# dusk-network/jubjub-schnorr

Measured on AMD Instinct MI355X. Metric: Schnorr verifications/sec, higher is better.
Workload: dtype u32 limbs (29-bit), u64 accumulators

## Files before the change

### jubjub_schnorr_amd/csrc/ed29.h

```cpp
#pragma once
#include "fq29.h"

namespace jjs {

using fe_t = fe<1, 5>;

struct ext_pt {
    fe_n x, y, z, t;
};
struct niels_pt {
    fe_t ypx, ymx, z, t2d;
};

JJS_HD fe_n fe_n_one() { return fq_as<1, 2>(fq_one()); }
JJS_HD fe_n fe_n_zero() { return fq_as<1, 2>(fq_zero()); }

JJS_HD ext_pt ext_identity() {
    ext_pt p;
    p.x = fe_n_zero(); p.y = fe_n_one(); p.z = fe_n_one(); p.t = fe_n_zero();
    return p;
}
JJS_HD ext_pt ext_from_affine(const fe_n& u, const fe_n& v) {
    ext_pt p;
    p.x = u; p.y = v; p.z = fe_n_one(); p.t = fq_mul(u, v);
    return p;
}
JJS_HD niels_pt niels_identity() {
    niels_pt n;
    n.ypx = fq_as<1, 5>(fq_one()); n.ymx = n.ypx; n.z = n.ypx; n.t2d = fq_as<1, 5>(fq_zero());
    return n;
}
JJS_HD niels_pt to_niels(const ext_pt& p) {
    niels_pt n;
    n.ypx = fq_as<1, 5>(fq_norm(fq_add(p.y, p.x)));
    n.ymx = fq_norm(fq_sub(p.y, p.x));
    n.z = fq_as<1, 5>(p.z);
    n.t2d = fq_as<1, 5>(fq_mul(p.t, fe_from_const<1, 1>(JJS_D2)));
    return n;
}
JJS_HD niels_pt niels_select(bool c, const niels_pt& a, const niels_pt& b) {
    niels_pt r;
    r.ypx = fq_select(c, a.ypx, b.ypx); r.ymx = fq_select(c, a.ymx, b.ymx);
    r.z = fq_select(c, a.z, b.z); r.t2d = fq_select(c, a.t2d, b.t2d);
    return r;
}

JJS_HD ext_pt ext_double(const ext_pt& p, bool need_t) {
    auto e = fq_dbl(fq_mul_hot(p.x, p.y));
    fe_n xx = fq_sqr_hot(p.x);
    fe_n yy = fq_sqr_hot(p.y);
    auto c2 = fq_dbl(fq_sqr_hot(p.z));
    auto g = fq_norm(fq_add(yy, xx));
    auto h = fq_sub(yy, xx);
    auto f = fq_norm(fq_sub(fq_add(c2, xx), yy));
    ext_pt r;
    r.x = fq_mul_hot(e, f);
    r.z = fq_mul_hot(f, h);
    r.y = fq_mul_hot(h, g);
    if (need_t) r.t = fq_mul_hot(g, e); else r.t = fe_n_zero();
    return r;
}

JJS_HD ext_pt ext_add_niels(const ext_pt& p, const niels_pt& n, bool neg, bool need_t) {
    fe_t n_ymx = fq_select(neg, n.ypx, n.ymx);
    fe_t n_ypx = fq_select(neg, n.ymx, n.ypx);
    auto n_t2d = fq_select(neg, fq_neg(n.t2d), fq_as<2, 6>(n.t2d));
    fe_n a = fq_mul_hot(fq_sub(p.y, p.x), n_ymx);
    fe_n b = fq_mul_hot(fq_add(p.y, p.x), n_ypx);
    fe_n c = fq_mul_hot(p.t, n_t2d);
    auto d = fq_dbl(fq_mul_hot(p.z, n.z));
    auto e = fq_sub(b, a);
    auto f = fq_norm(fq_sub(d, c));
    auto g = fq_add(d, c);
    auto h = fq_norm(fq_add(b, a));
    ext_pt r;
    r.x = fq_mul_hot(e, f);
    r.z = fq_mul_hot(f, g);
    r.y = fq_mul_hot(g, h);
    if (need_t) r.t = fq_mul_hot(h, e); else r.t = fe_n_zero();
    return r;
}
JJS_HD ext_pt ext_add_affine_niels(const ext_pt& p, const fe_t& n_ypx, const fe_t& n_ymx, const fe_t& n_t2d,
                                   bool need_t) {
    fe_n a = fq_mul_hot(fq_sub(p.y, p.x), n_ymx);
    fe_n b = fq_mul_hot(fq_add(p.y, p.x), n_ypx);
    fe_n c = fq_mul_hot(p.t, n_t2d);
    auto d = fq_dbl(p.z);
    auto e = fq_sub(b, a);
    auto f = fq_norm(fq_sub(d, c));
    auto g = fq_add(d, c);
    auto h = fq_norm(fq_add(b, a));
    ext_pt r;
    r.x = fq_mul_hot(e, f);
    r.z = fq_mul_hot(f, g);
    r.y = fq_mul_hot(g, h);
    if (need_t) r.t = fq_mul_hot(h, e); else r.t = fe_n_zero();
    return r;
}

JJS_HD bool ext_is_identity(const ext_pt& p) { return fq_is_zero(p.x) && fq_eq(p.y, p.z); }

JJS_HD bool affine_on_curve(const fe_n& u, const fe_n& v) {
    fe_n u2 = fq_sqr(u), v2 = fq_sqr(v);
    auto lhs = fq_sub(v2, u2);
    auto rhs = fq_norm(fq_add(fq_mul(fq_mul(u2, v2), fe_from_const<1, 1>(JJS_D)), fq_one()));
    return fq_eq(lhs, rhs);
}
JJS_HD bool affine_is_identity(const fe_n& u, const fe_n& v) { return fq_is_zero(u) && fq_eq(v, fq_one()); }

JJS_HD bool ext_eq_affine(const ext_pt& p, const fe_n& u, const fe_n& v) {
    return fq_eq(p.x, fq_mul(u, p.z)) && fq_eq(p.y, fq_mul(v, p.z));
}

}
```

### jubjub_schnorr_amd/csrc/jjs_constants.inc

```
#define JJS_MAX_HASH_INPUTS 16
#define JJS_Q29_0 0x00000001u
#define JJS_Q29_1 0x1ffffff8u
#define JJS_Q29_2 0x1f96ffbfu
#define JJS_Q29_3 0x1b4805ffu
#define JJS_Q29_4 0x1d80553bu
#define JJS_Q29_5 0x0c0404d0u
#define JJS_Q29_6 0x1520cce7u
#define JJS_Q29_7 0x0a6533afu
#define JJS_Q29_8 0x0073eda7u
JJS_CONST uint32_t JJS_Q_WORDS[8] = {0x00000001u, 0xffffffffu, 0xfffe5bfeu, 0x53bda402u, 0x09a1d805u, 0x3339d808u, 0x299d7d48u, 0x73eda753u};
JJS_CONST uint32_t JJS_QM2_WORDS[8] = {0xffffffffu, 0xfffffffeu, 0xfffe5bfeu, 0x53bda402u, 0x09a1d805u, 0x3339d808u, 0x299d7d48u, 0x73eda753u};
JJS_CONST uint32_t JJS_FR_WORDS[8] = {0xd6f72cb7u, 0xd0970e5eu, 0xccc81082u, 0xa6682093u, 0x01343b00u, 0x06673b01u, 0x6533afa9u, 0x0e7db4eau};
JJS_CONST uint32_t JJS_FR_R2_WORDS[8] = {0x95e57731u, 0x67719aa4u, 0x9ce3fc26u, 0x51b0cef0u, 0xc026e9a5u, 0x69dab7fau, 0x8d127688u, 0x04f6547bu};
#define JJS_FR_INV32 0xef788ef9u
JJS_CONST uint32_t JJS_R2[9] = {0x0a71b3c0u, 0x1d32207eu, 0x1663d999u, 0x1c5abc93u, 0x03b58c44u, 0x0be37438u, 0x0829f771u, 0x1660139eu, 0x0027fd91u};
JJS_CONST uint32_t JJS_ONE[9] = {0x1fffffbau, 0x0000022fu, 0x1cb61180u, 0x0a4e5c00u, 0x0ee8b1a2u, 0x16e6aedfu, 0x1907f8bbu, 0x0853ddf7u, 0x004d043fu};
JJS_CONST uint32_t JJS_D[9] = {0x0e9ed5e8u, 0x12245679u, 0x002d9f52u, 0x03bb3367u, 0x0d9bfb3du, 0x18ebb3ccu, 0x1c29ceccu, 0x0a7b6020u, 0x0020d725u};
JJS_CONST uint32_t JJS_D2[9] = {0x1d3dabd0u, 0x0448acf2u, 0x005b3ea5u, 0x077666ceu, 0x1b37f67au, 0x11d76798u, 0x18539d99u, 0x14f6c041u, 0x0041ae4au};
JJS_CONST uint32_t JJS_G[2][9] = {{0x0f8e352bu, 0x0d898cfcu, 0x1acf8b86u, 0x11cbaed5u, 0x11f53f06u, 0x1e102b0eu, 0x1a54d9c6u, 0x143eceffu, 0x006815d6u}, {0x1ffffb09u, 0x000027b7u, 0x09503dc0u, 0x0d6a3610u, 0x07d8d3d7u, 0x180c16bcu, 0x1a26af41u, 0x038c62dfu, 0x006f1642u}};
JJS_CONST uint32_t JJS_GN[2][9] = {{0x187d023du, 0x137e7289u, 0x0690434eu, 0x1f76361du, 0x00cee7a6u, 0x0f6ffe89u, 0x0eae76dcu, 0x0b002f63u, 0x001b3c2eu}, {0x0d19dfe5u, 0x1ba2bfe4u, 0x0aa87077u, 0x0a3c12aeu, 0x0f209d38u, 0x03331d80u, 0x05e964c7u, 0x046d436du, 0x00027722u}};
JJS_CONST uint32_t JJS_DOUBLE_TAG_WORDS[8] = {0x4844424cu, 0x4a4a5343u, 0x00000000u, 0x00000000u, 0x00000000u, 0x00000000u, 0x00000000u, 0x00000000u};
JJS_CONST uint32_t JJS_SPONGE_TAG[JJS_MAX_HASH_INPUTS + 1][9] = {
  {0x00000000u, 0x00000000u, 0x00000000u, 0x00000000u, 0x00000000u, 0x00000000u, 0x00000000u, 0x00000000u, 0x00000000u},
  {0x0505ee08u, 0x1a263c20u, 0x0be84b8bu, 0x14a02c49u, 0x01c71b32u, 0x0119871du, 0x0e158ab3u, 0x1ae4f29eu, 0x002534dfu},
  {0x1b0be909u, 0x1f0bd4a7u, 0x15c76ef6u, 0x19aa6651u, 0x03d277dau, 0x02c51eb8u, 0x131e6edfu, 0x1c823839u, 0x0028ae1cu},
  {0x0fc46418u, 0x0273db7eu, 0x16529079u, 0x104dd318u, 0x168e8637u, 0x026f5725u, 0x1c808eacu, 0x029e0e17u, 0x003fedbdu},
  {0x0357c163u, 0x10043808u, 0x19bdf7a6u, 0x0d30d38fu, 0x12e5297bu, 0x1c58dc5fu, 0x0ba83205u, 0x06d45679u, 0x00090830u},
  {0x0262554eu, 0x06977c58u, 0x1cc4c932u, 0x13bcc122u, 0x0d7d7321u, 0x16c6f8cdu, 0x0c42072du, 0x0a7ba9d5u, 0x00467f10u},
  {0x16ed364au, 0x0b0ae88eu, 0x1bd377f9u, 0x1bebcca6u, 0x0fbf0111u, 0x0eacca90u, 0x174be582u, 0x0d8cb0dfu, 0x006048a8u},
  {0x1648d83cu, 0x1c96a336u, 0x13f93121u, 0x0404c2c5u, 0x12088053u, 0x05063ca4u, 0x1387a958u, 0x0e2ca8b5u, 0x000dc63bu},
  {0x1f8df888u, 0x05a7ef5au, 0x1e8dea4fu, 0x04cf9c40u, 0x03a338cdu, 0x11ce25feu, 0x08f757fcu, 0x197c5746u, 0x00448b3du},
  {0x18861d85u, 0x0bfc90f3u, 0x01a0c7f1u, 0x0b8f8540u, 0x061d8364u, 0x17492b24u, 0x1f89fbceu, 0x03e0f6e4u, 0x002d13cau},
  {0x0f24fc1du, 0x17584430u, 0x197f7236u, 0x1bad9229u, 0x17ce7252u, 0x12745987u, 0x119f85a5u, 0x0365f792u, 0x00419641u},
  {0x0ad4ee1du, 0x1c33dd77u, 0x03cea63au, 0x0090b229u, 0x1eff0500u, 0x1ae3d4a9u, 0x0e58224eu, 0x1ba57ecau, 0x00131c30u},
  {0x0047e885u, 0x12b591deu, 0x09f50887u, 0x0c3877f6u, 0x01adcabbu, 0x00dcbf79u, 0x0ac6f554u, 0x0bcc64deu, 0x0062115cu},
  {0x18868630u, 0x0c3e88d9u, 0x0d12f54du, 0x062083b4u, 0x00efbe4eu, 0x1c915ba8u, 0x11f90d73u, 0x1200490cu, 0x00205cd9u},
  {0x109c52e0u, 0x100352e0u, 0x0d1863ecu, 0x0f9203ccu, 0x08db7deau, 0x1ea7d49cu, 0x0641cbbeu, 0x1693107au, 0x00056607u},
  {0x07380761u, 0x0379c563u, 0x10c89db4u, 0x0924fcebu, 0x0cf29ce1u, 0x1bfecb19u, 0x1a3ca913u, 0x12d81574u, 0x0008852cu},
  {0x0137f8a1u, 0x135b43b9u, 0x1a25c48fu, 0x04e620e0u, 0x0f670a49u, 0x190a832du, 0x1c3afc44u, 0x0c7a93dbu, 0x0026b4abu},
};
JJS_CONST uint32_t JJS_PAIR_L1[2][9] = {{0x1632f828u, 0x1cd998edu, 0x06ef42eau, 0x18522084u, 0x12362748u, 0x02a698c9u, 0x1b29c579u, 0x021b0691u, 0x003c41f3u}, {0x1b06fde4u, 0x137cdc5cu, 0x1714b9b2u, 0x065d7f7du, 0x140f3e68u, 0x08fb5d4bu, 0x18ad857au, 0x02b255c2u, 0x005ac97bu}};
JJS_CONST uint32_t JJS_PAIR_NEG_L2[9] = {0x0ec609f6u, 0x0fa98aa5u, 0x012a02e2u, 0x17e06bfeu, 0x14bb44c6u, 0x0c66138cu, 0x166a4edbu, 0x0ffd0b0au, 0x0050cfe0u};
JJS_CONST uint32_t JJS_PAIR_B[9] = {0x002c2b67u, 0x1e9ea4c8u, 0x07b6263fu, 0x1afbd911u, 0x133cdbc5u, 0x16559828u, 0x1a61d3c3u, 0x10975a2au, 0x00520471u};
JJS_CONST uint32_t JJS_PAIR_EXP_WORDS[8] = {0xe0000000u, 0xdfffffffu, 0x5fffcb7fu, 0xaa77b480u, 0x01343b00u, 0x06673b01u, 0x6533afa9u, 0x0e7db4eau};
#define JJS_PAIR_SW_STEPS 57
#define JJS_PAIR_SW_TRAILING 29
JJS_CONST uint32_t JJS_PAIR_SW[JJS_PAIR_SW_STEPS][2] = {{3, 7}, {5, 7}, {2, 3}, {3, 3}, {3, 3}, {2, 1}, {5, 7}, {4, 5}, {4, 3}, {5, 5}, {4, 3}, {5, 7}, {4, 5}, {3, 7}, {3, 5}, {2, 1}, {3, 1}, {7, 3}, {4, 3}, {5, 7}, {5, 7}, {3, 3}, {8, 1}, {8, 1}, {4, 3}, {2, 1}, {7, 7}, {3, 3}, {11, 5}, {4, 5}, {5, 7}, {4, 7}, {3, 5}, {3, 5}, {3, 1}, {11, 5}, {3, 7}, {3, 7}, {3, 7}, {3, 7}, {2, 3}, {5, 5}, {3, 5}, {3, 7}, {3, 7}, {2, 3}, {4, 7}, {3, 7}, {3, 7}, {3, 7}, {3, 7}, {3, 7}, {3, 7}, {3, 7}, {3, 7}, {3, 7}, {2, 3}};
#define JJS_INV_SW_STEPS 68
#define JJS_INV_SW_TRAILING 0
JJS_CONST uint32_t JJS_INV_SW[JJS_INV_SW_STEPS][2] = {{3, 7}, {5, 7}, {2, 3}, {3, 3}, {3, 3}, {2, 1}, {5, 7}, {4, 5}, {4, 3}, {5, 5}, {4, 3}, {5, 7}, {4, 5}, {3, 7}, {3, 5}, {2, 1}, {3, 1}, {7, 3}, {4, 3}, {5, 7}, {5, 7}, {3, 3}, {8, 1}, {8, 1}, {4, 3}, {2, 1}, {7, 7}, {3, 3}, {11, 5}, {4, 5}, {5, 7}, {4, 7}, {3, 5}, {3, 5}, {3, 1}, {11, 5}, {3, 7}, {3, 7}, {3, 7}, {3, 7}, {2, 3}, {5, 5}, {3, 5}, {3, 7}, {3, 7}, {2, 3}, {4, 7}, {3, 7}, {3, 7}, {3, 7}, {3, 7}, {3, 7}, {3, 7}, {3, 7}, {3, 7}, {3, 7}, {3, 5}, {3, 7}, {3, 7}, {3, 7}, {3, 7}, {3, 7}, {3, 7}, {3, 7}, {3, 7}, {3, 7}, {3, 7}, {1, 1}};
#define JJS_SQRT_SW_STEPS 57
#define JJS_SQRT_SW_TRAILING 0
JJS_CONST uint32_t JJS_SQRT_SW[JJS_SQRT_SW_STEPS][2] = {{3, 7}, {5, 7}, {2, 3}, {3, 3}, {3, 3}, {2, 1}, {5, 7}, {4, 5}, {4, 3}, {5, 5}, {4, 3}, {5, 7}, {4, 5}, {3, 7}, {3, 5}, {2, 1}, {3, 1}, {7, 3}, {4, 3}, {5, 7}, {5, 7}, {3, 3}, {8, 1}, {8, 1}, {4, 3}, {2, 1}, {7, 7}, {3, 3}, {11, 5}, {4, 5}, {5, 7}, {4, 7}, {3, 5}, {3, 5}, {3, 1}, {11, 5}, {3, 7}, {3, 7}, {3, 7}, {3, 7}, {2, 3}, {5, 5}, {3, 5}, {3, 7}, {3, 7}, {2, 3}, {4, 7}, {3, 7}, {3, 7}, {3, 7}, {3, 7}, {3, 7}, {3, 7}, {3, 7}, {3, 7}, {3, 7}, {1, 1}};
JJS_CONST uint32_t JJS_DLOG_BASES[7][9] = {{0x1e643334u, 0x16481b3cu, 0x1b429d12u, 0x177f9dadu, 0x144a8d18u, 0x0d45bdd8u, 0x04734720u, 0x08d7bfb9u, 0x0036d431u}, {0x015b5931u, 0x170bf111u, 0x0fdc692cu, 0x1da57375u, 0x1cd8fb0cu, 0x082b2e9eu, 0x11dae58du, 0x1c3e92cdu, 0x007386deu}, {0x046746cau, 0x011b8fe2u, 0x1ba33a6du, 0x176e1524u, 0x09d99e75u, 0x154d7d8eu, 0x00d23d31u, 0x1df2d37eu, 0x000963afu}, {0x1e643334u, 0x16481b3cu, 0x1b429d12u, 0x177f9dadu, 0x144a8d18u, 0x0d45bdd8u, 0x04734720u, 0x08d7bfb9u, 0x0036d431u}, {0x065b9ba7u, 0x16d68576u, 0x182b2c2au, 0x14d5af02u, 0x07140888u, 0x1362f1d7u, 0x08c77bb2u, 0x1cb1a9c5u, 0x00094bf1u}, {0x1abc62ceu, 0x0fbddb01u, 0x140b0090u, 0x03bc5521u, 0x11f8af58u, 0x1881ae47u, 0x11d5d43eu, 0x0a2d9980u, 0x005fe400u}, {0x04fbdc84u, 0x10c8e2ffu, 0x041d8af4u, 0x1a3da377u, 0x19ceef70u, 0x002b6e41u, 0x0034a007u, 0x1c185b28u, 0x0007ee60u}};
#define JJS_DLOG_HASH_MULT 1u
#define JJS_DLOG_HASH_SHIFT 0
JJS_CONST uint32_t JJS_ROOT_OF_UNITY[9] = {0x01c8cd27u, 0x158d8d27u, 0x19006c0du, 0x09177006u, 0x1b40635eu, 0x01d0b1cau, 0x0d517805u, 0x04859aa2u, 0x002c4064u};
JJS_CONST uint32_t JJS_RC[340][9] = {
  {0x00acd34au, 0x1735f45au, 0x138d6d99u, 0x0ed55d98u, 0x1ca62dc6u, 0x10ba9671u, 0x10435733u, 0x033b644du, 0x004aa8c7u},
  {0x14ffba26u, 0x1ba29e52u, 0x177f0b64u, 0x00b3510cu, 0x127726cfu, 0x1857d2a8u, 0x1e3d168au, 0x15e4d101u, 0x000f1ecau},
  {0x10544837u, 0x105827efu, 0x084c6e15u, 0x0e8aac41u, 0x0ae02b0fu, 0x18ebde5au, 0x0fafaf7cu, 0x083d3281u, 0x0034fd73u},
  {0x0344bf7fu, 0x0a46646au, 0x1730014du, 0x12e0ba85u, 0x02e3906cu, 0x05e7a406u, 0x17f2dc8bu, 0x1945722eu, 0x003a6ecfu},
  {0x1fd22f28u, 0x045b2ea8u, 0x17a649b2u, 0x0f9d7504u, 0x11961944u, 0x1660a34bu, 0x0a6a6237u, 0x193bc629u, 0x0021ffc7u},
  {0x1d29e5b8u, 0x06cae729u, 0x151ba656u, 0x1ac9f0b1u, 0x1b3a5e51u, 0x0d4ca236u, 0x1207ea27u, 0x1d21fa02u, 0x0022dd1fu},
  {0x12400ff9u, 0x0035d81du, 0x03b62299u, 0x025d538au, 0x08e06dddu, 0x1bbf452cu, 0x094dfd08u, 0x00285210u, 0x00308fabu},
  {0x1d184e77u, 0x1592ad1fu, 0x16661d64u, 0x1fe21660u, 0x1bfeebb3u, 0x0b7e4ad3u, 0x17ca297au, 0x15006fa8u, 0x001db197u},
  {0x1ddad3c4u, 0x13a1d246u, 0x071c897bu, 0x164f9a39u, 0x0689f7a5u, 0x080f8889u, 0x135aee92u, 0x03a580b3u, 0x006f4972u},
  {0x0d6eb0dbu, 0x058fde5bu, 0x1499b97cu, 0x0f49db3bu, 0x0ed02c77u, 0x0cd55fdeu, 0x029ef2fbu, 0x1f5282afu, 0x002a2cdcu},
  {0x1ab8ab5fu, 0x027938ecu, 0x0c556f7eu, 0x09fbfaf8u, 0x0ae0ef37u, 0x19cb8097u, 0x0358d657u, 0x12a3f282u, 0x002ebee0u},
  {0x12dd5a05u, 0x1eba6f91u, 0x00b2d3d3u, 0x0aa6ae2cu, 0x13721dbbu, 0x1619de12u, 0x0b03bb30u, 0x1947db06u, 0x000b396bu},
  {0x1f8c17c0u, 0x01352a93u, 0x09e2ed99u, 0x07dac2cdu, 0x0d3aedbeu, 0x053f5f63u, 0x1b33c7e7u, 0x10c2ba42u, 0x0057396bu},
  {0x0e64cfffu, 0x126637e6u, 0x1a0794f9u, 0x1d461805u, 0x01391d16u, 0x1546bc79u, 0x05f70070u, 0x07ffb18du, 0x001842b2u},
  {0x0e764d8au, 0x16095bb4u, 0x0eff26e0u, 0x0b91cc80u, 0x10ecd53du, 0x13e34450u, 0x0ded21a8u, 0x0a797e6eu, 0x00097bc9u},
  {0x1ea10b88u, 0x1f8971a2u, 0x12d7c69du, 0x1ebf9d1bu, 0x0901446fu, 0x001128c0u, 0x12fb8a56u, 0x062dd94au, 0x00133c86u},
  {0x0475856du, 0x0abc329fu, 0x15340d60u, 0x1aad5748u, 0x18d82c8eu, 0x112bd03fu, 0x0968aeabu, 0x1486dedeu, 0x00015fefu},
  {0x1d7537ecu, 0x074ba0f7u, 0x1a721561u, 0x0744501eu, 0x0b007d84u, 0x1f48b991u, 0x05982416u, 0x0db60c99u, 0x00640d9du},
  {0x0c0843e2u, 0x03da3b84u, 0x11b64327u, 0x1e4cf2b5u, 0x0362be93u, 0x073908a4u, 0x111e896bu, 0x19a5370bu, 0x0060b5a1u},
  {0x041c3708u, 0x15a529cau, 0x0af208bau, 0x059ec823u, 0x04adaedau, 0x1c9d2e20u, 0x161e5858u, 0x01c42fc5u, 0x00086bb0u},
  {0x07694f92u, 0x13ae592au, 0x1c584e2du, 0x0d28e81eu, 0x0e2c6ba5u, 0x00fe9197u, 0x1abf8e80u, 0x1a27fee9u, 0x00485be2u},
  {0x07317a6bu, 0x0fa6ca26u, 0x1c9ff3b6u, 0x04efe969u, 0x16037767u, 0x01818d54u, 0x0d467b33u, 0x1cf0127bu, 0x0012464fu},
  {0x1e8f2ddfu, 0x163c9dd6u, 0x054458f4u, 0x0b8d34b0u, 0x1569598au, 0x072ff89du, 0x01e3b883u, 0x1a85a626u, 0x0061760fu},
  {0x1dce8bb4u, 0x123fcb46u, 0x0377270du, 0x1ff43d6du, 0x09f2576fu, 0x063160f4u, 0x08fa3825u, 0x1d5b8f9fu, 0x00143750u},
  {0x0ca6e3c0u, 0x0be01d37u, 0x027fe433u, 0x0b5e8701u, 0x15745f3fu, 0x12446696u, 0x1792deb8u, 0x19ebb330u, 0x0028ae39u},
  {0x080574c2u, 0x1933ba92u, 0x07703651u, 0x024f101bu, 0x0d36f598u, 0x082ac40du, 0x1d43cc3bu, 0x08f57c17u, 0x004478e1u},
  {0x13e3176cu, 0x197fcd89u, 0x0d40b6d5u, 0x18c3e73cu, 0x0caa29f7u, 0x1a3dd941u, 0x0822f80du, 0x153d7eb4u, 0x0003f6bbu},
  {0x1133c83eu, 0x0561f86fu, 0x1495a2ecu, 0x08f377e4u, 0x1f9edff7u, 0x1b8e2211u, 0x0972815au, 0x1edeeea1u, 0x00528a97u},
  {0x040f1ff8u, 0x0d592276u, 0x1fd1391du, 0x06d2d8d0u, 0x173771ccu, 0x1091a88fu, 0x10c199d6u, 0x0744b505u, 0x00222937u},
  {0x1435b931u, 0x18719e1du, 0x15b840ddu, 0x1e6589bcu, 0x09af144fu, 0x1f4b724du, 0x188537c8u, 0x10bb12feu, 0x0025b1b9u},
  {0x18bcb3d3u, 0x113c16a2u, 0x00343982u, 0x1d45172cu, 0x1e078693u, 0x1eccfa04u, 0x06b5adbeu, 0x04fdea5cu, 0x0049ae25u},
  {0x0f642e85u, 0x117e9970u, 0x03334867u, 0x0dc3cd09u, 0x0e688815u, 0x01dafb58u, 0x0c65ac08u, 0x163dd834u, 0x003e51b1u},
  {0x076d4ca2u, 0x17a68f6cu, 0x17e794c3u, 0x0476c409u, 0x1dc62390u, 0x13fb540eu, 0x04377607u, 0x175fed3bu, 0x00673945u},
  {0x03d7a9a5u, 0x17067e90u, 0x0bbe3605u, 0x09fc7df9u, 0x084f4633u, 0x09c77039u, 0x085b07b0u, 0x1f974af1u, 0x000aa412u},
  {0x0006e8f6u, 0x11b32449u, 0x15d063e6u, 0x111532e4u, 0x01610a1bu, 0x18830975u, 0x037e3607u, 0x101e74c1u, 0x0025374cu},
  {0x1d91d5f1u, 0x0f1f6f98u, 0x11609817u, 0x008ea0beu, 0x00d542aeu, 0x03690ea1u, 0x1a69f7f8u, 0x07384443u, 0x004f4511u},
  {0x16b9fe96u, 0x1c99f301u, 0x098c16c4u, 0x12e36cf6u, 0x04a63222u, 0x18b5cb86u, 0x082733d6u, 0x081464b0u, 0x0015218du},
  {0x06e94ecbu, 0x0176fd7au, 0x011b1291u, 0x1b28987du, 0x0f265083u, 0x13440009u, 0x14b47c36u, 0x1a11baf7u, 0x00311fc6u},
  {0x1daafe06u, 0x114310cfu, 0x1f440ac5u, 0x1ab7d048u, 0x1c072ba7u, 0x103b3e08u, 0x0c6611c5u, 0x06b20990u, 0x00553a1fu},
  {0x00d69362u, 0x144b033du, 0x0df168b9u, 0x1c5d0c40u, 0x18666d4fu, 0x1a6ceafdu, 0x146c73a6u, 0x16cf5ea1u, 0x004cba1du},
  {0x1914c7dbu, 0x0d993b19u, 0x0b217f1fu, 0x104bc8f6u, 0x1e95409fu, 0x055c8f3du, 0x1cd77572u, 0x195653feu, 0x0013faddu},
  {0x1a5c25d7u, 0x0a07ef15u, 0x0a02d10bu, 0x03afd0a0u, 0x0af97875u, 0x150a4e2cu, 0x10c11760u, 0x13fa176eu, 0x00000329u},
  {0x1d7698b1u, 0x16f2d1c7u, 0x190ffc99u, 0x0a0bda41u, 0x194359f5u, 0x1574d2f3u, 0x0bd94f8au, 0x07464952u, 0x0019c91fu},
// ... 443 lines not shown
```

### jubjub_schnorr_amd/csrc/key_tables.h

```cpp
#pragma once
#include "verify_core.h"
#include "decode.h"
#include "ed29_quad.h"

namespace jjs {

constexpr int KT_WINDOW_NARROW = 5, KT_WINDOW_WIDE = 6;
constexpr uint32_t KT_WIDE_MULTIPLICITY = 128;
JJS_HD constexpr int kt_positions(int w) { return (252 + w) / w; }
JJS_HD constexpr int kt_entries(int w) { return (1 << (w - 1)) + 1; }
JJS_HD constexpr int kt_table_words(int w) { return kt_entries(w) * ENTRY_WORDS; }
constexpr int KT_MAX_POSITIONS = kt_positions(KT_WINDOW_NARROW);
static_assert(KT_WINDOW_NARROW >= 4 && KT_WINDOW_WIDE <= 6 && KT_WINDOW_NARROW < KT_WINDOW_WIDE, "digit extraction assumes a digit spans at most two words");
constexpr uint32_t KT_MIN_MULTIPLICITY = 16;
constexpr uint32_t KT_MAX_PROBES = 128;
constexpr uint32_t KT_KEY_MALFORMED = 1, KT_KEY_VALID = 2;
constexpr int KT_BASE_WORDS = 36;
JJS_HD constexpr size_t kt_max(size_t a, size_t b) { return a > b ? a : b; }
JJS_HD constexpr size_t kt_base_words_for_keys(size_t narrow, size_t wide) {
    return kt_max(narrow * kt_positions(KT_WINDOW_NARROW), wide * kt_positions(KT_WINDOW_WIDE)) * KT_BASE_WORDS;
}
JJS_HD constexpr size_t kt_table_words_for_keys(size_t narrow, size_t wide) {
    return kt_max(narrow * kt_positions(KT_WINDOW_NARROW) * kt_table_words(KT_WINDOW_NARROW),
                  wide * kt_positions(KT_WINDOW_WIDE) * kt_table_words(KT_WINDOW_WIDE));
// ... 120 lines not shown
    return valid;
}

#if defined(__HIPCC__)
__device__ __forceinline__ void kt_chain_key_quad(const key_column& C, uint32_t id, int w, uint32_t j) {
    const uint64_t item = C.key_item[id];
    const fe_n pu = fq_from_words(load_words(C.src, item)), pv = fq_from_words(load_words(C.src, item, 32));
    ext_pt p = ext_from_affine(pu, pv);
    if (j == 0) kt_store_ext(kt_base(C, id, 0, w), p);
    const uint32_t positions = (uint32_t)kt_positions(w);
    for (uint32_t pos = 1; pos < positions; ++pos) {
        fe_n own;
#pragma unroll 1
        for (int k = 0; k < w; ++k) p = ext_double_quad(p, j, own);
        uint32_t* dst = kt_base(C, id, pos, w) + 9 * j;
#pragma unroll
        for (int i = 0; i < 9; ++i) dst[i] = own.l[i];
    }
}
#endif
JJS_HD bool kt_key_flags(const key_column& C, uint32_t id) {
    const uint64_t item = C.key_item[id];
    const words8 uw = load_words(C.src, item), vw = load_words(C.src, item, 32);
    const bool canonical = words_lt(uw, JJS_Q_WORDS) && words_lt(vw, JJS_Q_WORDS);
    const fe_n pu = fq_from_words(uw), pv = fq_from_words(vw);
    const bool valid = canonical && point_on_curve_not_identity(pu, pv) && is_torsion_free(pu, pv);
    C.key_flags[id] = (uint8_t)((canonical ? 0u : KT_KEY_MALFORMED) | (valid ? KT_KEY_VALID : 0u));
    return valid;
}

JJS_HD void kt_build_table(uint32_t* tab, const ext_pt& p1, int entries) {
    const niels_pt n1 = to_niels(p1);
    store_niels(tab, niels_identity());
    store_niels(tab + ENTRY_WORDS, n1);
    ext_pt acc = ext_double(p1, true);
    store_niels(tab + 2 * ENTRY_WORDS, to_niels(acc));
    for (int j = 3; j < entries; ++j) {
        acc = ext_add_niels(acc, n1, false, true);
        store_niels(tab + j * ENTRY_WORDS, to_niels(acc));
    }
}
JJS_HD void kt_table_lane(const key_column& C, uint32_t id, uint32_t pos, int w) {
    kt_build_table(kt_table(C, id, pos, w), kt_load_ext(kt_base(C, id, pos, w)), kt_entries(w));
}

JJS_HD constexpr uint32_t kt_recode_word(int w, int word) {
    uint32_t v = 0;
    for (int i = 0; i < kt_positions(w) - 1; ++i) {
        const int bit = w * i + w - 1;
        if ((bit >> 5) == word) v |= 1u << (bit & 31);
    }
    return v;
}
JJS_HD words8 kt_recode(const words8& s, int w) {
    constexpr uint32_t KN[8] = {kt_recode_word(KT_WINDOW_NARROW, 0), kt_recode_word(KT_WINDOW_NARROW, 1), kt_recode_word(KT_WINDOW_NARROW, 2),
                                kt_recode_word(KT_WINDOW_NARROW, 3), kt_recode_word(KT_WINDOW_NARROW, 4), kt_recode_word(KT_WINDOW_NARROW, 5),
                                kt_recode_word(KT_WINDOW_NARROW, 6), kt_recode_word(KT_WINDOW_NARROW, 7)};
    constexpr uint32_t KW[8] = {kt_recode_word(KT_WINDOW_WIDE, 0), kt_recode_word(KT_WINDOW_WIDE, 1), kt_recode_word(KT_WINDOW_WIDE, 2),
                                kt_recode_word(KT_WINDOW_WIDE, 3), kt_recode_word(KT_WINDOW_WIDE, 4), kt_recode_word(KT_WINDOW_WIDE, 5),
                                kt_recode_word(KT_WINDOW_WIDE, 6), kt_recode_word(KT_WINDOW_WIDE, 7)};
    const bool wide = w == KT_WINDOW_WIDE;
    words8 r;
    uint64_t carry = 0;
#pragma unroll
    for (int i = 0; i < 8; ++i) {
        const uint64_t t = (uint64_t)s.w[i] + (wide ? KW[i] : KN[i]) + carry;
        r.w[i] = (uint32_t)t;
        carry = t >> 32;
    }
    return r;
}
JJS_HD ext_pt kt_add_digit(const ext_pt& acc, const uint32_t* tab, const words8& sc, int pos, int w) {
    const int bit = w * pos, wi = bit >> 5, sh = bit & 31;
    uint32_t v = word_at(sc, wi) >> sh;
    if (sh + w > 32) v |= word_at(sc, wi + 1 > 7 ? 7 : wi + 1) << (32 - sh);
    const uint32_t raw = v & ((1u << w) - 1u);
    const bool top = pos == kt_positions(w) - 1;
    const int d = top ? (int)(word_at(sc, wi) >> sh) : (int)raw - (1 << (w - 1));
    const bool neg = d < 0;
    uint32_t idx = (uint32_t)(neg ? -d : d);
    idx = idx >= (uint32_t)kt_entries(w) ? (uint32_t)kt_entries(w) - 1u : idx;
    return ext_add_niels(acc, load_niels(tab + idx * ENTRY_WORDS), neg, true);
}
JJS_HD ext_pt kt_add_scalar(ext_pt acc, const key_column& C, uint32_t id, const words8& s, int w) {
    const words8 sc = kt_recode(s, w);
    for (int pos = kt_positions(w) - 1; pos >= 0; --pos) acc = kt_add_digit(acc, kt_table(C, id, (uint32_t)pos, w), sc, pos, w);
    return acc;
}

JJS_HD uint32_t kt_finish_item(const verify_params& P, const key_params& K, uint64_t item, const prep_record& r) {
    const int w = (int)*P.key_flag;
    const words8 u = load_words(P.u, item);
    bool keys_valid = true, keys_malformed = false, eq_ok = true;
    for (uint32_t e = 0; e < P.n_eq; ++e) {
        const eq_desc& E = P.eq[e];
        ext_pt acc = ext_identity();
        {
            const key_column C = kt_col(K, E.pk_col);
            const uint32_t id = C.keyid[item], f = C.key_flags[id];
            keys_valid = keys_valid && (f & KT_KEY_VALID) != 0;
            keys_malformed = keys_malformed || (f & KT_KEY_MALFORMED) != 0;
            acc = kt_add_scalar(acc, C, id, r.c, w);
        }
        if (E.comb) {
            acc = add_comb(acc, E.comb, u, JJS_SKIP(P, 16u));
        } else {
            const key_column C = kt_col(K, E.gen_col);
            const uint32_t id = C.keyid[item], f = C.key_flags[id];
            keys_valid = keys_valid && (f & KT_KEY_VALID) != 0;
            keys_malformed = keys_malformed || (f & KT_KEY_MALFORMED) != 0;
            acc = kt_add_scalar(acc, C, id, u, w);
        }
        const fe_n ru = load_fq(E.r, item), rv = load_fq(E.r, item, 32);
        eq_ok = ext_eq_affine(acc, ru, rv) && eq_ok;
    }
    if (r.malformed || keys_malformed || !words_lt(u, JJS_FR_WORDS)) return ST_MALFORMED;
    if (!r.valid || !keys_valid) return ST_INVALID_POINT;
    if (JJS_SKIP(P, 1u)) return eq_ok ? ST_OK : ST_INVALID_SIGNATURE;
    return eq_ok ? ST_OK : ST_PENDING_EQ_FAILED;
}

}
```

### jubjub_schnorr_amd/csrc/verify_core.h

```cpp
#pragma once
#include <cmath>

#include "ed29.h"
#include "hades29.h"
#include "fq_inv.h"

namespace jjs {

enum : uint32_t { ST_OK = 0, ST_INVALID_POINT = 1, ST_INVALID_SIGNATURE = 2, ST_MALFORMED = 3 };
enum : uint32_t { ST_PENDING_EQ_FAILED = 4, ST_PENDING_EQ_HELD = 5 };

struct fe_src {
    const uint8_t* base;
    uint32_t stride;
    uint32_t off;
};
struct eq_desc {
    const uint32_t* comb;
    fe_src gen;
    fe_src pk;
    fe_src r;
    int32_t pk_col, gen_col;
};
struct verify_params {
// ... 372 lines not shown
            shl_words(x, k);
            shl_words(y, k);
        }
        uint32_t q = (uint32_t)qd;
        q = q ? q : 1u;
        q = single ? q : 0u;
        uint32_t n0[8], m0[4];
        uint64_t carry = 0;
        uint32_t borrow = 0;
#pragma unroll
        for (int i = 0; i < 8; ++i) {
            carry += (uint64_t)q * x[i];
            uint64_t d = (uint64_t)r0[i] - (uint32_t)carry - borrow;
            n0[i] = (uint32_t)d;
            borrow = (uint32_t)(d >> 63);
            carry >>= 32;
        }
        carry = 0;
#pragma unroll
        for (int i = 0; i < 4; ++i) {
            carry += (uint64_t)q * y[i] + t0[i];
            m0[i] = (uint32_t)carry;
            carry >>= 32;
        }
        const bool swap = single && lt_words(n0, r1);
#pragma unroll
        for (int i = 0; i < 8; ++i) {
            const uint32_t a = n0[i], b = r1[i];
            r0[i] = swap ? b : a;
            r1[i] = swap ? a : b;
        }
#pragma unroll
        for (int i = 0; i < 4; ++i) {
            const uint32_t a = m0[i], b = t1[i];
            t0[i] = swap ? b : a;
            t1[i] = swap ? a : b;
        }
        neg = swap ? !neg : neg;
    }
    half_scalars h;
#pragma unroll
    for (int i = 0; i < 4; ++i) { h.a.w[i] = r1[i]; h.b.w[i] = t1[i]; }
    h.b_neg = neg;
    return h;
}

JJS_HD bool is_torsion_free_by_order(const fe_n& u, const fe_n& v) {
    ext_pt p = ext_from_affine(u, v);
    niels_pt n = to_niels(p);
    ext_pt acc = p;
    for (int i = 250; i >= 0; --i) {
        bool bit = (JJS_FR_WORDS[i >> 5] >> (i & 31)) & 1;
        acc = ext_double(acc, bit);
        if (bit) acc = ext_add_affine_niels(acc, n.ypx, n.ymx, n.t2d, false);
    }
    return ext_is_identity(acc);
}

JJS_HD bool pairing_is_trivial(const fe_n& px, const fe_n& py, const fe_n& pz) {
    auto opv = fq_add(pz, py);
    auto omv = fq_sub(pz, py);
    fe_n w = fq_mul(omv, px);
    fe_n x = fq_mul(opv, px);
    fe_n oz = fq_mul(opv, pz);
    fe_n xw[2] = {x, w};
    auto l1 = fq_norm(fq_add(oz, fq_dot_const<2, 2>(JJS_PAIR_L1, xw)));
    auto l2 = fq_norm(fq_add(oz, fq_mul(x, fe_from_const<1, 1>(JJS_PAIR_NEG_L2))));
    auto vv = fq_norm(fq_sub(x, w));
    fe_n a = fq_mul(fq_sqr(l1), l2);
    a = fq_sqr(fq_mul(a, fq_sqr(vv)));
    fe_n y = fq_mul(fq_mul(x, w), fe_from_const<1, 1>(JJS_PAIR_B));
    fe_n y2 = fq_sqr(y);
    fe_n y7 = fq_mul(fq_mul(fq_sqr(y2), y2), y);
    fe_n g = fq_mul(a, y7);
    fe_n e = fq_pow_schedule(g, JJS_PAIR_SW, JJS_PAIR_SW_STEPS, JJS_PAIR_SW_TRAILING);
    return fq_eq(e, fq_one());
}
JJS_HD bool is_torsion_free(const fe_n& u, const fe_n& v) { return pairing_is_trivial(u, v, fe_n_one()); }

JJS_HD bool point_on_curve_not_identity(const fe_n& u, const fe_n& v) {
    return affine_on_curve(u, v) && !affine_is_identity(u, v);
}

JJS_HD ext_pt add_comb_range(ext_pt acc, const uint32_t* comb, const words8& k, int lo, int hi, bool t_last,
                             bool one_entry = false) {
    for (int i = lo; i < hi; ++i) {
        constexpr int per_word = 32 / COMB_BITS;
        uint32_t digit = (word_at(k, i / per_word) >> ((i % per_word) * COMB_BITS)) & (uint32_t)(COMB_ENTRIES - 1);
        digit = one_entry ? (digit & 255u) : digit;
        const u32x4* p = reinterpret_cast<const u32x4*>(comb + ((size_t)i * COMB_ENTRIES + digit) * COMB_ENTRY_WORDS);
        uint32_t w[COMB_ENTRY_WORDS];
#pragma unroll
        for (int k4 = 0; k4 < COMB_ENTRY_WORDS / 4; ++k4) { u32x4 v = p[k4]; w[4 * k4] = v.x; w[4 * k4 + 1] = v.y; w[4 * k4 + 2] = v.z; w[4 * k4 + 3] = v.w; }
        fe_t ypx, ymx, t2d;
#pragma unroll
        for (int j = 0; j < 9; ++j) { ypx.l[j] = w[j]; ymx.l[j] = w[9 + j]; t2d.l[j] = w[18 + j]; }
        acc = ext_add_affine_niels(acc, ypx, ymx, t2d, t_last || i != hi - 1);
    }
    return acc;
}
JJS_HD ext_pt add_comb(ext_pt acc, const uint32_t* comb, const words8& k, bool one_entry = false) {
    return add_comb_range(acc, comb, k, 0, COMB_WINDOWS, false, one_entry);
}
JJS_HD words8 widen128(const u128w& x) {
    words8 r;
#pragma unroll
    for (int i = 0; i < 8; ++i) r.w[i] = i < 4 ? x.w[i] : 0u;
    return r;
}
JJS_HD words8 recode_signed4_128(const u128w& s) {
    words8 r;
    uint64_t carry = 0;
#pragma unroll
    for (int i = 0; i < 8; ++i) {
        uint64_t t = (uint64_t)(i < 4 ? s.w[i] : 0u) + (i < 3 ? 0x88888888u : (i == 3 ? 0x08888888u : 0u)) + carry;
        r.w[i] = (uint32_t)t;
        carry = t >> 32;
    }
    return r;
}

JJS_HD words8 select_words(bool c, const words8& a, const words8& b) {
    words8 r;
#pragma unroll
    for (int i = 0; i < 8; ++i) r.w[i] = c ? a.w[i] : b.w[i];
    return r;
}

JJS_HD words8 half_scalar_times_u(const half_scalars& h, const words8& u) {
    words8 r2;
#pragma unroll
    for (int i = 0; i < 8; ++i) r2.w[i] = JJS_FR_R2_WORDS[i];
    words8 w = fr_mont_mul(fr_mont_mul(widen128(h.b), r2), u);
    uint32_t nz = 0, borrow = 0;
    words8 n;
#pragma unroll
    for (int i = 0; i < 8; ++i) {
        nz |= w.w[i];
        uint64_t d = (uint64_t)JJS_FR_WORDS[i] - w.w[i] - borrow;
        n.w[i] = (uint32_t)d;
        borrow = (uint32_t)(d >> 63);
    }
    return select_words(h.b_neg && nz != 0, n, w);
}

JJS_HD bool check_equation(const eq_desc& E, uint64_t item, uint32_t* ws, const words8& u, const words8& c,
                           const half_scalars& h, const uint32_t* shared_tab = nullptr) {
    const bool one_entry = shared_tab != nullptr;
    const bool fixed = (E.comb != nullptr);
#pragma unroll 1
    for (int t = 0; t < 2; ++t) {
        const fe_src& src = (t == 0) ? E.pk : (fixed ? E.r : E.gen);
        fe_n pu = load_fq(src, item), pv = load_fq(src, item, 32);
        build_point_table(ws + t * TABLE_WORDS, pu, pv);
    }
    words8 s0, s1, w;
    int top;
    bool flip1;
    if (fixed) {
        w = half_scalar_times_u(h, u);
        s0 = recode_signed4_128(h.a);
        s1 = recode_signed4_128(h.b);
        top = 31;
        flip1 = !h.b_neg;
    } else {
        s0 = recode_signed4(c);
        s1 = recode_signed4(u);
        w = u;
        top = 63;
        flip1 = false;
    }
    ext_pt acc = ext_identity();
    for (int win = top; win >= 0; --win) {
        if (win != top) {
#pragma unroll 1
            for (int j = 0; j < 4; ++j) acc = ext_double(acc, j == 3);
        }
#pragma unroll 1
        for (int t = 0; t < 2; ++t) {
            const words8 sc = select_words(t == 0, s0, s1);
// ... 185 lines not shown
```

Measured before the change: 117.8 million.

## Prefetch table entries ahead of point additions and skip work for invalid waves

The comb and key-table accumulation loops now load the next table entry before running the current point addition, so global memory latency can overlap with field arithmetic. Digit extraction is reworked into a shifting register window, which avoids dynamic indexing into the scalar words. The first two key-table additions from the identity are merged into one niels+niels sum that uses an inverse-2d constant, saving a multiply chain. The full verification is skipped when every lane in a wave is malformed or invalid. In exchange, the prefetch buffers raise register pressure and may lower occupancy.

```diff
diff --git a/jubjub_schnorr_amd/csrc/ed29.h b/jubjub_schnorr_amd/csrc/ed29.h
--- a/jubjub_schnorr_amd/csrc/ed29.h
+++ b/jubjub_schnorr_amd/csrc/ed29.h
@@ -61,14 +61,7 @@
     return r;
 }
 
-JJS_HD ext_pt ext_add_niels(const ext_pt& p, const niels_pt& n, bool neg, bool need_t) {
-    fe_t n_ymx = fq_select(neg, n.ypx, n.ymx);
-    fe_t n_ypx = fq_select(neg, n.ymx, n.ypx);
-    auto n_t2d = fq_select(neg, fq_neg(n.t2d), fq_as<2, 6>(n.t2d));
-    fe_n a = fq_mul_hot(fq_sub(p.y, p.x), n_ymx);
-    fe_n b = fq_mul_hot(fq_add(p.y, p.x), n_ypx);
-    fe_n c = fq_mul_hot(p.t, n_t2d);
-    auto d = fq_dbl(fq_mul_hot(p.z, n.z));
+JJS_HD ext_pt ext_add_finish(const fe_n& a, const fe_n& b, const fe_n& c, const fe<2, 4>& d, bool need_t) {
     auto e = fq_sub(b, a);
     auto f = fq_norm(fq_sub(d, c));
     auto g = fq_add(d, c);
@@ -79,6 +72,27 @@
     r.y = fq_mul_hot(g, h);
     if (need_t) r.t = fq_mul_hot(h, e); else r.t = fe_n_zero();
     return r;
+}
+JJS_HD ext_pt ext_add_niels(const ext_pt& p, const niels_pt& n, bool neg, bool need_t) {
+    fe_t n_ymx = fq_select(neg, n.ypx, n.ymx);
+    fe_t n_ypx = fq_select(neg, n.ymx, n.ypx);
+    auto n_t2d = fq_select(neg, fq_neg(n.t2d), fq_as<2, 6>(n.t2d));
+    fe_n a = fq_mul_hot(fq_sub(p.y, p.x), n_ymx);
+    fe_n b = fq_mul_hot(fq_add(p.y, p.x), n_ypx);
+    fe_n c = fq_mul_hot(p.t, n_t2d);
+    auto d = fq_dbl(fq_mul_hot(p.z, n.z));
+    return ext_add_finish(a, b, c, d, need_t);
+}
+JJS_HD ext_pt ext_niels_sum(const niels_pt& n1, bool neg1, const niels_pt& n2, bool neg2, bool need_t) {
+    const fe_t ymx1 = fq_select(neg1, n1.ypx, n1.ymx), ypx1 = fq_select(neg1, n1.ymx, n1.ypx);
+    const fe_t ymx2 = fq_select(neg2, n2.ypx, n2.ymx), ypx2 = fq_select(neg2, n2.ymx, n2.ypx);
+    const auto t2d1 = fq_select(neg1, fq_neg(n1.t2d), fq_as<2, 6>(n1.t2d));
+    const auto t2d2 = fq_select(neg2, fq_neg(n2.t2d), fq_as<2, 6>(n2.t2d));
+    fe_n a = fq_mul_hot(ymx1, ymx2);
+    fe_n b = fq_mul_hot(ypx1, ypx2);
+    fe_n c = fq_mul_hot(fq_mul(t2d1, fe_from_const<1, 1>(JJS_INV_D2)), t2d2);
+    auto d = fq_dbl(fq_mul_hot(n1.z, n2.z));
+    return ext_add_finish(a, b, c, d, need_t);
 }
 JJS_HD ext_pt ext_add_affine_niels(const ext_pt& p, const fe_t& n_ypx, const fe_t& n_ymx, const fe_t& n_t2d,
                                    bool need_t) {
diff --git a/jubjub_schnorr_amd/csrc/jjs_constants.inc b/jubjub_schnorr_amd/csrc/jjs_constants.inc
--- a/jubjub_schnorr_amd/csrc/jjs_constants.inc
+++ b/jubjub_schnorr_amd/csrc/jjs_constants.inc
@@ -17,6 +17,7 @@
 JJS_CONST uint32_t JJS_ONE[9] = {0x1fffffbau, 0x0000022fu, 0x1cb61180u, 0x0a4e5c00u, 0x0ee8b1a2u, 0x16e6aedfu, 0x1907f8bbu, 0x0853ddf7u, 0x004d043fu};
 JJS_CONST uint32_t JJS_D[9] = {0x0e9ed5e8u, 0x12245679u, 0x002d9f52u, 0x03bb3367u, 0x0d9bfb3du, 0x18ebb3ccu, 0x1c29ceccu, 0x0a7b6020u, 0x0020d725u};
 JJS_CONST uint32_t JJS_D2[9] = {0x1d3dabd0u, 0x0448acf2u, 0x005b3ea5u, 0x077666ceu, 0x1b37f67au, 0x11d76798u, 0x18539d99u, 0x14f6c041u, 0x0041ae4au};
+JJS_CONST uint32_t JJS_INV_D2[9] = {0x13333357u, 0x1ffffee1u, 0x04842a3fu, 0x0a45a399u, 0x002584f8u, 0x07c312d1u, 0x1ac9745bu, 0x0dc0a0c3u, 0x0035d599u};
 JJS_CONST uint32_t JJS_G[2][9] = {{0x0f8e352bu, 0x0d898cfcu, 0x1acf8b86u, 0x11cbaed5u, 0x11f53f06u, 0x1e102b0eu, 0x1a54d9c6u, 0x143eceffu, 0x006815d6u}, {0x1ffffb09u, 0x000027b7u, 0x09503dc0u, 0x0d6a3610u, 0x07d8d3d7u, 0x180c16bcu, 0x1a26af41u, 0x038c62dfu, 0x006f1642u}};
 JJS_CONST uint32_t JJS_GN[2][9] = {{0x187d023du, 0x137e7289u, 0x0690434eu, 0x1f76361du, 0x00cee7a6u, 0x0f6ffe89u, 0x0eae76dcu, 0x0b002f63u, 0x001b3c2eu}, {0x0d19dfe5u, 0x1ba2bfe4u, 0x0aa87077u, 0x0a3c12aeu, 0x0f209d38u, 0x03331d80u, 0x05e964c7u, 0x046d436du, 0x00027722u}};
 JJS_CONST uint32_t JJS_DOUBLE_TAG_WORDS[8] = {0x4844424cu, 0x4a4a5343u, 0x00000000u, 0x00000000u, 0x00000000u, 0x00000000u, 0x00000000u, 0x00000000u};
diff --git a/jubjub_schnorr_amd/csrc/key_tables.h b/jubjub_schnorr_amd/csrc/key_tables.h
--- a/jubjub_schnorr_amd/csrc/key_tables.h
+++ b/jubjub_schnorr_amd/csrc/key_tables.h
@@ -226,10 +226,77 @@
     idx = idx >= (uint32_t)kt_entries(w) ? (uint32_t)kt_entries(w) - 1u : idx;
     return ext_add_niels(acc, load_niels(tab + idx * ENTRY_WORDS), neg, true);
 }
-JJS_HD ext_pt kt_add_scalar(ext_pt acc, const key_column& C, uint32_t id, const words8& s, int w) {
-    const words8 sc = kt_recode(s, w);
-    for (int pos = kt_positions(w) - 1; pos >= 0; --pos) acc = kt_add_digit(acc, kt_table(C, id, (uint32_t)pos, w), sc, pos, w);
+struct kt_digits {
+    uint32_t v[9];
+    int base;
+};
+JJS_HD kt_digits kt_digits_of(const words8& sc) {
+    kt_digits d;
+#pragma unroll
+    for (int i = 0; i < 8; ++i) d.v[i] = sc.w[i];
+    d.v[8] = 0;
+    d.base = 224;
+    return d;
+}
+JJS_HD uint32_t kt_bits_at(kt_digits& d, int bit) {
+    if (bit < d.base) {
+#pragma unroll
+        for (int i = 8; i > 0; --i) d.v[i] = d.v[i - 1];
+        d.v[0] = 0;
+        d.base -= 32;
+    }
+    return (uint32_t)((((uint64_t)d.v[8] << 32) | d.v[7]) >> (uint32_t)(bit - d.base));
+}
+struct kt_entry {
+    const uint32_t* p;
+    bool neg;
+};
+JJS_HD kt_entry kt_entry_at(const key_column& C, uint32_t id, kt_digits& dg, int pos, int w) {
+    const uint32_t bits = kt_bits_at(dg, w * pos);
+    const bool top = pos == kt_positions(w) - 1;
+    const int d = top ? (int)(bits & (0xffffffffu >> ((w * pos) & 31))) : (int)(bits & ((1u << w) - 1u)) - (1 << (w - 1));
+    const bool neg = d < 0;
+    uint32_t idx = (uint32_t)(neg ? -d : d);
+    idx = idx >= (uint32_t)kt_entries(w) ? (uint32_t)kt_entries(w) - 1u : idx;
+    return kt_entry{kt_table(C, id, (uint32_t)pos, w) + idx * ENTRY_WORDS, neg};
+}
+JJS_HD ext_pt kt_add_scalar(ext_pt acc, const key_column& C, uint32_t id, const words8& s, int w, bool fresh = false) {
+    kt_digits dg = kt_digits_of(kt_recode(s, w));
+    int pos = kt_positions(w) - 1;
+    kt_entry e = kt_entry_at(C, id, dg, pos, w);
+    niels_pt cur = load_niels(e.p);
+    bool neg = e.neg;
+    if (fresh) {
+        e = kt_entry_at(C, id, dg, pos - 1, w);
+        const niels_pt second = load_niels(e.p);
+        const bool second_neg = e.neg;
+        pos -= 2;
+        e = kt_entry_at(C, id, dg, pos, w);
+        const niels_pt next = load_niels(e.p);
+        acc = ext_niels_sum(cur, neg, second, second_neg, true);
+        cur = next;
+        neg = e.neg;
+    }
+    for (; pos >= 1; pos -= 2) {
+        e = kt_entry_at(C, id, dg, pos - 1, w);
+        const niels_pt second = load_niels(e.p);
+        const bool second_neg = e.neg;
+        acc = ext_add_niels(acc, cur, neg, true);
+        e = kt_entry_at(C, id, dg, pos >= 2 ? pos - 2 : 0, w);
+        cur = load_niels(e.p);
+        neg = e.neg;
+        acc = ext_add_niels(acc, second, second_neg, true);
+    }
+    if (pos == 0) acc = ext_add_niels(acc, cur, neg, true);
     return acc;
+}
+
+JJS_HD bool kt_wave_all(bool pred) {
+#if defined(__HIP_DEVICE_COMPILE__)
+    return __all(pred) != 0;
+#else
+    return pred;
+#endif
 }
 
 JJS_HD uint32_t kt_finish_item(const verify_params& P, const key_params& K, uint64_t item, const prep_record& r) {
@@ -238,27 +305,33 @@
     bool keys_valid = true, keys_malformed = false, eq_ok = true;
     for (uint32_t e = 0; e < P.n_eq; ++e) {
         const eq_desc& E = P.eq[e];
-        ext_pt acc = ext_identity();
-        {
-            const key_column C = kt_col(K, E.pk_col);
-            const uint32_t id = C.keyid[item], f = C.key_flags[id];
+        for (int g = 0; g < (E.comb ? 1 : 2); ++g) {
+            const key_column C = kt_col(K, g == 0 ? E.pk_col : E.gen_col);
+            const uint32_t f = C.key_flags[C.keyid[item]];
             keys_valid = keys_valid && (f & KT_KEY_VALID) != 0;
             keys_malformed = keys_malformed || (f & KT_KEY_MALFORMED) != 0;
-            acc = kt_add_scalar(acc, C, id, r.c, w);
         }
-        if (E.comb) {
-            acc = add_comb(acc, E.comb, u, JJS_SKIP(P, 16u));
-        } else {
-            const key_column C = kt_col(K, E.gen_col);
-            const uint32_t id = C.keyid[item], f = C.key_flags[id];
-            keys_valid = keys_valid && (f & KT_KEY_VALID) != 0;
-            keys_malformed = keys_malformed || (f & KT_KEY_MALFORMED) != 0;
-            acc = kt_add_scalar(acc, C, id, u, w);
+    }
+    const bool malformed = r.malformed || keys_malformed || !words_lt(u, JJS_FR_WORDS);
+    if (!kt_wave_all(malformed || !r.valid || !keys_valid)) {
+        for (uint32_t e = 0; e < P.n_eq; ++e) {
+            const eq_desc& E = P.eq[e];
+            ext_pt acc;
+            {
+                const key_column C = kt_col(K, E.pk_col);
+                acc = kt_add_scalar(ext_identity(), C, C.keyid[item], r.c, w, true);
+            }
+            if (E.comb) {
+                acc = add_comb(acc, E.comb, u, JJS_SKIP(P, 16u));
+            } else {
+                const key_column C = kt_col(K, E.gen_col);
+                acc = kt_add_scalar(acc, C, C.keyid[item], u, w);
+            }
+            const fe_n ru = load_fq(E.r, item), rv = load_fq(E.r, item, 32);
+            eq_ok = ext_eq_affine(acc, ru, rv) && eq_ok;
         }
-        const fe_n ru = load_fq(E.r, item), rv = load_fq(E.r, item, 32);
-        eq_ok = ext_eq_affine(acc, ru, rv) && eq_ok;
-    }
-    if (r.malformed || keys_malformed || !words_lt(u, JJS_FR_WORDS)) return ST_MALFORMED;
+    }
+    if (malformed) return ST_MALFORMED;
     if (!r.valid || !keys_valid) return ST_INVALID_POINT;
     if (JJS_SKIP(P, 1u)) return eq_ok ? ST_OK : ST_INVALID_SIGNATURE;
     return eq_ok ? ST_OK : ST_PENDING_EQ_FAILED;
diff --git a/jubjub_schnorr_amd/csrc/verify_core.h b/jubjub_schnorr_amd/csrc/verify_core.h
--- a/jubjub_schnorr_amd/csrc/verify_core.h
+++ b/jubjub_schnorr_amd/csrc/verify_core.h
@@ -478,20 +478,51 @@
     return affine_on_curve(u, v) && !affine_is_identity(u, v);
 }
 
+struct comb_digits {
+    uint32_t v[8];
+    int word;
+};
+JJS_HD comb_digits comb_digits_of(const words8& k) {
+    comb_digits d;
+#pragma unroll
+    for (int i = 0; i < 8; ++i) d.v[i] = k.w[i];
+    d.word = 0;
+    return d;
+}
+JJS_HD uint32_t comb_digit_at(comb_digits& d, int i) {
+    constexpr int per_word = 32 / COMB_BITS;
+    while (d.word < i / per_word) {
+#pragma unroll
+        for (int j = 0; j < 7; ++j) d.v[j] = d.v[j + 1];
+        d.v[7] = 0;
+        ++d.word;
+    }
+    return (d.v[0] >> ((i % per_word) * COMB_BITS)) & (uint32_t)(COMB_ENTRIES - 1);
+}
+struct comb_entry {
+    fe_t ypx, ymx, t2d;
+};
+JJS_HD comb_entry load_comb_entry(const uint32_t* comb, int i, uint32_t digit) {
+    const u32x4* p = reinterpret_cast<const u32x4*>(comb + ((size_t)i * COMB_ENTRIES + digit) * COMB_ENTRY_WORDS);
+    uint32_t w[COMB_ENTRY_WORDS];
+#pragma unroll
+    for (int k4 = 0; k4 < COMB_ENTRY_WORDS / 4; ++k4) { u32x4 v = p[k4]; w[4 * k4] = v.x; w[4 * k4 + 1] = v.y; w[4 * k4 + 2] = v.z; w[4 * k4 + 3] = v.w; }
+    comb_entry e;
+#pragma unroll
+    for (int j = 0; j < 9; ++j) { e.ypx.l[j] = w[j]; e.ymx.l[j] = w[9 + j]; e.t2d.l[j] = w[18 + j]; }
+    return e;
+}
 JJS_HD ext_pt add_comb_range(ext_pt acc, const uint32_t* comb, const words8& k, int lo, int hi, bool t_last,
                              bool one_entry = false) {
+    if (lo >= hi) return acc;
+    comb_digits dg = comb_digits_of(k);
+    const uint32_t sel = one_entry ? 255u : (uint32_t)(COMB_ENTRIES - 1);
+    comb_entry cur = load_comb_entry(comb, lo, comb_digit_at(dg, lo) & sel);
     for (int i = lo; i < hi; ++i) {
-        constexpr int per_word = 32 / COMB_BITS;
-        uint32_t digit = (word_at(k, i / per_word) >> ((i % per_word) * COMB_BITS)) & (uint32_t)(COMB_ENTRIES - 1);
-        digit = one_entry ? (digit & 255u) : digit;
-        const u32x4* p = reinterpret_cast<const u32x4*>(comb + ((size_t)i * COMB_ENTRIES + digit) * COMB_ENTRY_WORDS);
-        uint32_t w[COMB_ENTRY_WORDS];
-#pragma unroll
-        for (int k4 = 0; k4 < COMB_ENTRY_WORDS / 4; ++k4) { u32x4 v = p[k4]; w[4 * k4] = v.x; w[4 * k4 + 1] = v.y; w[4 * k4 + 2] = v.z; w[4 * k4 + 3] = v.w; }
-        fe_t ypx, ymx, t2d;
-#pragma unroll
-        for (int j = 0; j < 9; ++j) { ypx.l[j] = w[j]; ymx.l[j] = w[9 + j]; t2d.l[j] = w[18 + j]; }
-        acc = ext_add_affine_niels(acc, ypx, ymx, t2d, t_last || i != hi - 1);
+        comb_entry next = cur;
+        if (i + 1 < hi) next = load_comb_entry(comb, i + 1, comb_digit_at(dg, i + 1) & sel);
+        acc = ext_add_affine_niels(acc, cur.ypx, cur.ymx, cur.t2d, t_last || i != hi - 1);
+        cur = next;
     }
     return acc;
 }
```

Result: no change. 117.8 million, median of 6 (+0.0%).
